# liudabao001/JABD-Joint-Attention-Based-Detector-for-small-face-detection

Measured on AMD Instinct MI355X. Metric: images/sec at 1024x1024 bs32 (1/2/4/8 GPU); boxes/sec NMS, higher is better.
Workload: dtype fp32; 1 GPU; C2: JABD-MobileNetV3 RetinaFace (nets/retinaface_r.py) eval forward, weights_init weights; global_batch=32, image_size=1024, parallelism=replicas x1

## Files before the change

jabd-joint-attention-based-detector-for-small-face-detection_amd/csrc/conv32.hip:

```cpp
#include <stdlib.h>

#include <algorithm>
#include <type_traits>

#include "common.h"
#include "conv_args.h"

namespace jabd {

typedef float f32x16 __attribute__((ext_vector_type(16)));

__device__ __forceinline__ float act32(float v, int act, float slope) {
  switch (act) {
    case ACT_RELU: return relu_f(v);
    case ACT_LEAKY: return v > 0.f ? v : v * slope;
    case ACT_HSWISH: return hswish_f(v);
    case ACT_HSIGMOID: return hsigmoid_f(v);
    case ACT_SIGMOID: return 1.f / (1.f + expf(-v));
    default: return v;
  }
}

constexpr int kBK = 32;

__device__ __forceinline__ void wave_lds_sync32() {
  asm volatile("s_waitcnt lgkmcnt(0)" ::: "memory");
  __builtin_amdgcn_wave_barrier();
}
constexpr int kG = kBK / 8;
constexpr int kGateLds = 1024;

constexpr int kEpiPitch = 36;
enum { kEpiRt = 0, kEpiNone = 1, kEpiRes = 2 };
template <int TN, bool ST, bool BB, int EPI = kEpiRt>
__device__ __forceinline__ void m32_epilogue_tm1(const ConvArgs& p, const f32x16 (&acc)[TN],
                                                 int pm, int om, int nb, int srow, float* ep,
                                                 float* __restrict__ part, const BnEpi& bb,
                                                 int lane, int ch0 = 0) {
  const bool has_bias = EPI == kEpiRt && p.bias;
  const bool has_res = EPI == kEpiRes || (EPI == kEpiRt && p.res);
  const int h = lane >> 5, j = lane & 31;
  const int ep_px = lane >> 3, ep_q = lane & 7;
  int mrow[4], prow[4];
#pragma unroll
  for (int r = 0; r < 4; ++r) {
    prow[r] = __shfl(pm, ep_px + 8 * r);
    mrow[r] = __shfl(om, ep_px + 8 * r);
  }
#pragma unroll
  for (int u = 0; u < TN; ++u) {
    const int nb0 = (nb * TN + u) * 32 + ch0;
    if (nb0 >= p.Cout) break;
    const int n = nb0 + 4 * ep_q;
    float4 ss = make_float4(0.f, 0.f, 0.f, 0.f), sq = ss, sh = ss;
    float4 bmu = sh, bis = sh, bgm = sh, bbt = sh;
    float4 bx[4], bmk[4];
    if constexpr (BB) {
      if (n < p.Cout) {
        bmu = *reinterpret_cast<const float4*>(bb.mean + n);
        bis = *reinterpret_cast<const float4*>(bb.invstd + n);
        if (!bb.mask) {
          bgm = *reinterpret_cast<const float4*>(bb.gamma + n);
          bbt = *reinterpret_cast<const float4*>(bb.beta + n);
        }
      }
#pragma unroll
      for (int r = 0; r < 4; ++r)
        bx[r] = (prow[r] >= 0 && n < p.Cout)
                    ? *reinterpret_cast<const float4*>(bb.x + (int64_t)mrow[r] * bb.x_ps + n)
                    : sh;
      if (bb.mask) {
#pragma unroll
        for (int r = 0; r < 4; ++r)
          bmk[r] = (prow[r] >= 0 && n < p.Cout)
                       ? *reinterpret_cast<const float4*>(bb.mask + (int64_t)mrow[r] * bb.mask_ps + n)
                       : sh;
      }
    }
#pragma unroll
    for (int c = 0; c < 4; ++c)
      *reinterpret_cast<float4*>(ep + j * kEpiPitch + 8 * c + 4 * h) =
          make_float4(acc[u][4 * c], acc[u][4 * c + 1], acc[u][4 * c + 2],
                      acc[u][4 * c + 3]);
    wave_lds_sync32();
    if constexpr (ST) sh = *reinterpret_cast<const float4*>(ep + 4 * ep_q);
#pragma unroll
    for (int r = 0; r < 4; ++r) {
      const int px = ep_px + 8 * r;
      if (prow[r] < 0 || n >= p.Cout) continue;
      float4 v = *reinterpret_cast<const float4*>(ep + px * kEpiPitch + 4 * ep_q);
      if (BB && bb.mask) {
        if (p.res) {
          const float4 rr = *reinterpret_cast<const float4*>(p.res + (int64_t)mrow[r] * p.res_ps +
                                                             p.res_c0 + n);
          v.x += rr.x; v.y += rr.y; v.z += rr.z; v.w += rr.w;
        }
        v.x *= bmk[r].x > 0.f ? 1.f : 0.f;
        v.y *= bmk[r].y > 0.f ? 1.f : 0.f;
        v.z *= bmk[r].z > 0.f ? 1.f : 0.f;
        v.w *= bmk[r].w > 0.f ? 1.f : 0.f;
        const float xh0 = (bx[r].x - bmu.x) * bis.x, xh1 = (bx[r].y - bmu.y) * bis.y;
        const float xh2 = (bx[r].z - bmu.z) * bis.z, xh3 = (bx[r].w - bmu.w) * bis.w;
        ss.x += v.x; ss.y += v.y; ss.z += v.z; ss.w += v.w;
        sq.x += v.x * xh0; sq.y += v.y * xh1; sq.z += v.z * xh2; sq.w += v.w * xh3;
        *reinterpret_cast<float4*>(p.y + (int64_t)mrow[r] * p.y_ps + p.y_c0 + n) = v;
        continue;
      }
      if constexpr (BB) {
        const float xv[4] = {bx[r].x, bx[r].y, bx[r].z, bx[r].w};
        const float mu[4] = {bmu.x, bmu.y, bmu.z, bmu.w}, is[4] = {bis.x, bis.y, bis.z, bis.w};
        const float gm[4] = {bgm.x, bgm.y, bgm.z, bgm.w}, bt[4] = {bbt.x, bbt.y, bbt.z, bbt.w};
        const float gv[4] = {v.x, v.y, v.z, v.w};
        float dzs[4], dzx[4];
#pragma unroll
        for (int e = 0; e < 4; ++e) {
          const float xh = (xv[e] - mu[e]) * is[e];
          const float z = fmaf(xh, gm[e], bt[e]);
          const float d = bb.act == ACT_RELU ? (z > 0.f ? 1.f : 0.f)
                          : bb.act == ACT_LEAKY ? (z > 0.f ? 1.f : bb.slope) : 1.f;
          dzs[e] = gv[e] * d;
          dzx[e] = dzs[e] * xh;
        }
        ss.x += dzs[0]; ss.y += dzs[1]; ss.z += dzs[2]; ss.w += dzs[3];
        sq.x += dzx[0]; sq.y += dzx[1]; sq.z += dzx[2]; sq.w += dzx[3];
      }
      if constexpr (ST) {
        const float dx = v.x - sh.x, dy = v.y - sh.y, dz = v.z - sh.z, dw = v.w - sh.w;
        ss.x += dx; ss.y += dy; ss.z += dz; ss.w += dw;
        sq.x = fmaf(dx, dx, sq.x); sq.y = fmaf(dy, dy, sq.y);
        sq.z = fmaf(dz, dz, sq.z); sq.w = fmaf(dw, dw, sq.w);
      }
      if (has_bias) {
        const float4 bb = *reinterpret_cast<const float4*>(p.bias + n);
        v.x += bb.x; v.y += bb.y; v.z += bb.z; v.w += bb.w;
      }
      if (has_res) {
        const float4 rr = *reinterpret_cast<const float4*>(p.res + (int64_t)mrow[r] * p.res_ps +
                                                           p.res_c0 + n);
        v.x += rr.x; v.y += rr.y; v.z += rr.z; v.w += rr.w;
      }
      if constexpr (EPI == kEpiRt) {
        v.x = act32(v.x, p.act, p.slope);
        v.y = act32(v.y, p.act, p.slope);
        v.z = act32(v.z, p.act, p.slope);
        v.w = act32(v.w, p.act, p.slope);
      }
      *reinterpret_cast<float4*>(p.y + (int64_t)mrow[r] * p.y_ps + p.y_c0 + n) = v;
    }
    if constexpr (BB) {
#pragma unroll
      for (int off = 8; off <= 32; off <<= 1) {
        ss.x += __shfl_xor(ss.x, off); ss.y += __shfl_xor(ss.y, off);
        ss.z += __shfl_xor(ss.z, off); ss.w += __shfl_xor(ss.w, off);
        sq.x += __shfl_xor(sq.x, off); sq.y += __shfl_xor(sq.y, off);
        sq.z += __shfl_xor(sq.z, off); sq.w += __shfl_xor(sq.w, off);
      }
      if (ep_px == 0 && (int64_t)srow * 32 < p.M && n < p.Cout) {
        const int ldc = p.Ntiles * 32;
        float* pr = bb.rows + (int64_t)srow * 2 * ldc + n;
        *reinterpret_cast<float4*>(pr) = ss;
        *reinterpret_cast<float4*>(pr + ldc) = sq;
      }
    }
    if constexpr (ST) {
#pragma unroll
      for (int off = 8; off <= 32; off <<= 1) {
        ss.x += __shfl_xor(ss.x, off); ss.y += __shfl_xor(ss.y, off);
        ss.z += __shfl_xor(ss.z, off); ss.w += __shfl_xor(ss.w, off);
        sq.x += __shfl_xor(sq.x, off); sq.y += __shfl_xor(sq.y, off);
        sq.z += __shfl_xor(sq.z, off); sq.w += __shfl_xor(sq.w, off);
      }
      const int64_t cnt = min<int64_t>(32, p.M - (int64_t)srow * 32);
      if (ep_px == 0 && cnt > 0 && n < p.Cout) {
        const float inv = 1.f / (float)cnt;
        const int ldc = p.Ntiles * 32;
        float* pr = part + (int64_t)srow * 2 * ldc + n;
        *reinterpret_cast<float4*>(pr) =
            make_float4(fmaf(ss.x, inv, sh.x), fmaf(ss.y, inv, sh.y), fmaf(ss.z, inv, sh.z),
                        fmaf(ss.w, inv, sh.w));
        *reinterpret_cast<float4*>(pr + ldc) =
            make_float4(fmaxf(sq.x - ss.x * ss.x * inv, 0.f), fmaxf(sq.y - ss.y * ss.y * inv, 0.f),
                        fmaxf(sq.z - ss.z * ss.z * inv, 0.f), fmaxf(sq.w - ss.w * ss.w * inv, 0.f));
      }
    }
    wave_lds_sync32();
  }
}

enum { kSrcRt = 0, kSrcOne = 1, kSrcTwo = 2 };
template <int TM, int TN, bool KXK, bool AS, bool ST = false, bool BB = false, int EPI = kEpiRt,
          int SRC = kSrcRt>
__global__ __launch_bounds__(256, 2) void conv1x1_m32_kernel(const ConvArgs p, int mtiles_img,
                                                             int per_img, int phase, int ks,
                                                             float* __restrict__ part,
                                                             const BnEpi bb) {
  constexpr bool FAST = SRC != kSrcRt;
  static_assert(!FAST || (AS && !KXK), "SRC: the gated 1x1 forms only");
  constexpr int BM = 4 * 32 * TM;
  constexpr int NB4 = kG * TN * 64;
  constexpr int NBT = (NB4 + 255) / 256;
  constexpr int kEpi4 = 4 * 32 * kEpiPitch / 4;
  constexpr int SB4 = (TM == 1 && kEpi4 > 2 * NB4) ? kEpi4 : 2 * NB4;
  __shared__ float4 sB_[SB4];
  float4 (*sB)[NB4] = reinterpret_cast<float4 (*)[NB4]>(sB_);
  __shared__ __attribute__((aligned(16))) float sGate[AS ? kGateLds : 4];
  const int lane = threadIdx.x & 63, wave = threadIdx.x >> 6;
  const int h = lane >> 5, j = lane & 31;
  const int nblk_n = p.Ntiles / TN;
  const int bid = blockIdx.x;
  const int nb = bid % nblk_n, mb = bid / nblk_n;
  const int OHW = p.OH * p.OW;
  const int ph = phase >> 1, pw = phase & 1;
  const int SH = phase >= 0 ? (p.OH - ph + 1) >> 1 : p.OH;
  const int SW = phase >= 0 ? (p.OW - pw + 1) >> 1 : p.OW;
  const int kh0 = phase >= 0 ? (ph + p.pad) & 1 : 0, kw0 = phase >= 0 ? (pw + p.pad) & 1 : 0;
  const int nkh = phase >= 0 ? (p.KH - kh0 + 1) >> 1 : p.KH;
  const int nkw = phase >= 0 ? (p.KW - kw0 + 1) >> 1 : p.KW;
  const int M = phase >= 0 ? p.B * SH * SW : (int)p.M;
  int img = 0, m_lo, m_hi;
  if (per_img) {
    img = mb / mtiles_img;
    m_lo = img * OHW + (mb - img * mtiles_img) * BM;
    m_hi = min(img * OHW + OHW, M);
  } else {
    m_lo = mb * BM;
    m_hi = M;
  }
  int pm[TM];
#pragma unroll
  for (int t = 0; t < TM; ++t) {
    const int m = m_lo + wave * 32 * TM + t * 32 + j;
    pm[t] = m < m_hi ? m : -1;
  }
  const int Kt = KXK ? nkh * nkw * p.Cin
                     : p.Cin + ((FAST ? SRC == kSrcTwo : p.x2 != nullptr) ? p.Cin2 : 0);
  const int S_all = (Kt + kBK - 1) / kBK;
  const int kchunk = (S_all + ks - 1) / ks;
  const int s_beg = ks > 1 ? (int)blockIdx.y * kchunk : 0;
  const int S = ks > 1 ? min(S_all, s_beg + kchunk) : S_all;
  int poh[TM], pow_[TM], om[TM];
  int64_t pbase[TM];
#pragma unroll
  for (int t = 0; t < TM; ++t) om[t] = pm[t];
  if constexpr (KXK) {
#pragma unroll
    for (int t = 0; t < TM; ++t) {
      const int m = pm[t] >= 0 ? pm[t] : 0;
      const int SHW = SH * SW;
      const int b = m / SHW, r = m - b * SHW;
      const int i = r / SW, jj = r - i * SW;
      poh[t] = phase >= 0 ? 2 * i + ph : i;
      pow_[t] = phase >= 0 ? 2 * jj + pw : jj;
      pbase[t] = (int64_t)b * p.x_bs + p.x_c0;
      if (pm[t] >= 0) om[t] = (b * p.OH + poh[t]) * p.OW + pow_[t];
    }
  }
  const int cps = p.Cin / kBK;
  const int x2_pix = (p.x2 && p.x2_stride != 1) ? (int)(p.x2_bs / p.x2_ps) : 0;
  const float4* wg = reinterpret_cast<const float4*>(p.w);
  const float* sc = AS ? p.ascale + (int64_t)img * p.ascale_bs : nullptr;

  const float* xa[TM];
  const float* xb[TM];
  if constexpr (FAST) {
#pragma unroll
    for (int t = 0; t < TM; ++t) {
      const int ml = pm[t] >= 0 ? pm[t] : m_lo;
      xa[t] = p.x + (int64_t)ml * p.x_ps + p.x_c0;
      xb[t] = SRC == kSrcTwo ? p.x2 + (int64_t)ml * p.x2_ps - p.Cin : xa[t];
    }
  }
  auto load_a = [&](int s, float4 (&a)[TM][kG]) {
    if constexpr (FAST) {
#pragma unroll
      for (int t = 0; t < TM; ++t)
#pragma unroll
        for (int q = 0; q < kG; ++q) {
          const int k4 = min(s * kBK + 8 * q + 4 * h, Kt - 4);
          const float* src = (SRC == kSrcTwo && k4 >= p.Cin) ? xb[t] + k4 : xa[t] + k4;
          a[t][q] = *reinterpret_cast<const float4*>(src);
        }
      return;
    }
    if constexpr (KXK) {
      const int tl = s / cps, ci0 = (s - tl * cps) * kBK;
      const int khi = tl / nkw;
      const int kh = kh0 + (phase >= 0 ? 2 : 1) * khi;
      const int kw = kw0 + (phase >= 0 ? 2 : 1) * (tl - khi * nkw);
#pragma unroll
      for (int t = 0; t < TM; ++t) {
        const int ih = p.tconv ? (poh[t] + p.pad - kh) >> (phase >= 0 ? 1 : 0)
                               : poh[t] * p.stride - p.pad + kh;
        const int iw = p.tconv ? (pow_[t] + p.pad - kw) >> (phase >= 0 ? 1 : 0)
                               : pow_[t] * p.stride - p.pad + kw;
        const bool ok = pm[t] >= 0 && ih >= 0 && ih < p.H && iw >= 0 && iw < p.W;
        const float* src = p.x + pbase[t] + ((int64_t)ih * p.W + iw) * p.x_ps + ci0 + 4 * h;
#pragma unroll
        for (int q = 0; q < kG; ++q)
          a[t][q] = ok ? *reinterpret_cast<const float4*>(src + 8 * q)
                       : make_float4(0.f, 0.f, 0.f, 0.f);
      }
      return;
    }
#pragma unroll
    for (int t = 0; t < TM; ++t)
#pragma unroll
      for (int q = 0; q < kG; ++q) {
        const int k4 = s * kBK + 8 * q + 4 * h;
        const int m = pm[t];
        float4 r = make_float4(0.f, 0.f, 0.f, 0.f);
        if (m >= 0) {
          if (k4 < p.Cin) {
            r = *reinterpret_cast<const float4*>(p.x + (int64_t)m * p.x_ps + p.x_c0 + k4);
          } else if (k4 < Kt) {
            int qq = m;
            if (p.x2_stride != 1) {
              const int b = m / OHW, rr = m - b * OHW;
              const int oh = rr / p.OW, ow = rr - oh * p.OW;
              qq = b * x2_pix + (oh * p.x2_stride) * p.x2_W + ow * p.x2_stride;
            }
            r = *reinterpret_cast<const float4*>(p.x2 + (int64_t)qq * p.x2_ps + (k4 - p.Cin));
          }
        }
        a[t][q] = r;
      }
  };
  const bool gate_lds = FAST || (AS && p.Cin <= kGateLds);
  auto zero_tail = [&](int s, float4 (&a)[TM][kG]) {
    if (!FAST || (s + 1) * kBK <= Kt) return;
#pragma unroll
    for (int t = 0; t < TM; ++t)
#pragma unroll
      for (int q = 0; q < kG; ++q)
        if (s * kBK + 8 * q + 4 * h >= Kt) a[t][q] = make_float4(0.f, 0.f, 0.f, 0.f);
  };
  auto load_b = [&](int s, float4 (&b)[NBT]) {
    if (KXK && phase >= 0) {
      const int tl = s / cps, khi = tl / nkw;
      const int tap = (kh0 + 2 * khi) * p.KW + kw0 + 2 * (tl - khi * nkw);
      s = tap * cps + (s - tl * cps);
    }
#pragma unroll
    for (int i = 0; i < NBT; ++i) {
      const int f = i * 256 + threadIdx.x;
      float4 v = make_float4(0.f, 0.f, 0.f, 0.f);
      if (f < NB4) {
        const int g = f / (TN * 64), rem = f - g * (TN * 64);
        const int u = rem >> 6, l = rem & 63;
        const int k8 = s * kG + g;
        v = wg[((int64_t)k8 * p.Ntiles + nb * TN + u) * 64 + l];
        if (!FAST && sc && !gate_lds) {
          int k0 = 8 * k8 + 4 * (l >> 5);
          if (KXK) k0 -= (s / cps) * p.Cin;
          if (k0 < p.Cin) {
            const float4 s4 = *reinterpret_cast<const float4*>(sc + k0);
            v.x *= s4.x; v.y *= s4.y; v.z *= s4.z; v.w *= s4.w;
          }
        }
      }
      b[i] = v;
    }
  };
  auto store_b = [&](int buf, int s, const float4 (&b)[NBT]) {
    if (KXK && phase >= 0) {
      const int tl = s / cps, khi = tl / nkw;
      const int tap = (kh0 + 2 * khi) * p.KW + kw0 + 2 * (tl - khi * nkw);
      s = tap * cps + (s - tl * cps);
    }
#pragma unroll
    for (int i = 0; i < NBT; ++i) {
      const int f = i * 256 + threadIdx.x;
      if (f < NB4) {
        float4 v = b[i];
        if (gate_lds) {
          const int g = f / (TN * 64), l = f & 63;
          int k0 = 8 * (s * kG + g) + 4 * (l >> 5);
          if (KXK) k0 -= (s / cps) * p.Cin;
          if (k0 < p.Cin) {
            const float4 s4 = *reinterpret_cast<const float4*>(sGate + k0);
            v.x *= s4.x; v.y *= s4.y; v.z *= s4.z; v.w *= s4.w;
          }
        }
        sB[buf][f] = v;
      }
    }
  };

  f32x16 acc[TM][TN];
#pragma unroll
  for (int t = 0; t < TM; ++t)
#pragma unroll
    for (int u = 0; u < TN; ++u)
#pragma unroll
      for (int r = 0; r < 16; ++r) acc[t][u][r] = 0.f;

  float4 a_cur[TM][kG], a_nxt[TM][kG], b_nxt[NBT];
  if (gate_lds) {
    for (int i = threadIdx.x; i < p.Cin; i += 256) sGate[i] = sc[i];
    __syncthreads();
  }
  if (S > s_beg) {
    load_a(s_beg, a_cur);
    load_b(s_beg, b_nxt);
    store_b(s_beg & 1, s_beg, b_nxt);
    zero_tail(s_beg, a_cur);
  }
  __syncthreads();
  for (int s = s_beg; s < S; ++s) {
    const bool more = s + 1 < S;
    if (more) {
      load_a(s + 1, a_nxt);
      load_b(s + 1, b_nxt);
    }
    const float4* bs = sB[s & 1];
#pragma unroll
    for (int q = 0; q < kG; ++q) {
      float4 bw[TN];
#pragma unroll
      for (int u = 0; u < TN; ++u) bw[u] = bs[(q * TN + u) * 64 + lane];
#pragma unroll
      for (int t = 0; t < TM; ++t)
#pragma unroll
        for (int u = 0; u < TN; ++u)
          acc[t][u] = __builtin_amdgcn_mfma_f32_32x32x2f32(bw[u].x, a_cur[t][q].x, acc[t][u], 0, 0, 0);
#pragma unroll
      for (int t = 0; t < TM; ++t)
#pragma unroll
        for (int u = 0; u < TN; ++u)
          acc[t][u] = __builtin_amdgcn_mfma_f32_32x32x2f32(bw[u].y, a_cur[t][q].y, acc[t][u], 0, 0, 0);
#pragma unroll
      for (int t = 0; t < TM; ++t)
#pragma unroll
        for (int u = 0; u < TN; ++u)
          acc[t][u] = __builtin_amdgcn_mfma_f32_32x32x2f32(bw[u].z, a_cur[t][q].z, acc[t][u], 0, 0, 0);
#pragma unroll
      for (int t = 0; t < TM; ++t)
#pragma unroll
        for (int u = 0; u < TN; ++u)
          acc[t][u] = __builtin_amdgcn_mfma_f32_32x32x2f32(bw[u].w, a_cur[t][q].w, acc[t][u], 0, 0, 0);
    }
    if (more) {
      store_b((s + 1) & 1, s + 1, b_nxt);
#pragma unroll
      for (int t = 0; t < TM; ++t)
#pragma unroll
        for (int q = 0; q < kG; ++q) a_cur[t][q] = a_nxt[t][q];
      zero_tail(s + 1, a_cur);
    }
    __syncthreads();
  }

  if (ks > 1) {
    const int npad = p.Ntiles * 32;
    float* pb = part + (int64_t)blockIdx.y * p.M * npad;
#pragma unroll
    for (int t = 0; t < TM; ++t) {
      if (pm[t] < 0) continue;
      float* prow = pb + (int64_t)om[t] * npad;
#pragma unroll
      for (int u = 0; u < TN; ++u)
#pragma unroll
        for (int c = 0; c < 4; ++c) {
          const int n = (nb * TN + u) * 32 + 8 * c + 4 * h;
          *reinterpret_cast<float4*>(prow + n) = make_float4(
              acc[t][u][4 * c], acc[t][u][4 * c + 1], acc[t][u][4 * c + 2], acc[t][u][4 * c + 3]);
        }
    }
    return;
  }
  if constexpr (TM == 1) {
    float* ep = reinterpret_cast<float*>(sB_) + wave * 32 * kEpiPitch;
    const int srow = mb * 4 + wave;
    m32_epilogue_tm1<TN, ST, BB, (ST || BB) ? kEpiNone : EPI>(p, acc[0], pm[0], om[0], nb, srow,
                                                                ep, part, bb, lane);
    return;
  }
#pragma unroll
  for (int t = 0; t < TM; ++t) {
    const int m = om[t];
    if (pm[t] < 0) continue;
    float* yrow = p.y + (int64_t)m * p.y_ps + p.y_c0;
    const float* rrow = p.res ? p.res + (int64_t)m * p.res_ps + p.res_c0 : nullptr;
#pragma unroll
    for (int u = 0; u < TN; ++u)
#pragma unroll
      for (int c = 0; c < 4; ++c) {
        const int n = (nb * TN + u) * 32 + 8 * c + 4 * h;
        if (n >= p.Cout) continue;
        float4 v = make_float4(acc[t][u][4 * c], acc[t][u][4 * c + 1], acc[t][u][4 * c + 2],
                               acc[t][u][4 * c + 3]);
        if (p.bias) {
          const float4 bb = *reinterpret_cast<const float4*>(p.bias + n);
          v.x += bb.x; v.y += bb.y; v.z += bb.z; v.w += bb.w;
        }
        if (rrow) {
          const float4 rr = *reinterpret_cast<const float4*>(rrow + n);
          v.x += rr.x; v.y += rr.y; v.z += rr.z; v.w += rr.w;
        }
        v.x = act32(v.x, p.act, p.slope);
        v.y = act32(v.y, p.act, p.slope);
        v.z = act32(v.z, p.act, p.slope);
        v.w = act32(v.w, p.act, p.slope);
        *reinterpret_cast<float4*>(yrow + n) = v;
      }
  }

}

__global__ __launch_bounds__(256) void m32_ksplit_reduce(const ConvArgs p, int ks,
                                                         const float* __restrict__ part) {
  const int npad = p.Ntiles * 32, c4n = (p.Cout + 3) >> 2;
  const int64_t i = blockIdx.x * (int64_t)blockDim.x + threadIdx.x;
  if (i >= p.M * c4n) return;
  const int64_t m = i / c4n;
  const int n = (int)(i - m * c4n) * 4;
  float4 v = *reinterpret_cast<const float4*>(part + m * npad + n);
  for (int y = 1; y < ks; ++y) {
    const float4 q = *reinterpret_cast<const float4*>(part + ((int64_t)y * p.M + m) * npad + n);
    v.x += q.x; v.y += q.y; v.z += q.z; v.w += q.w;
  }
  if (p.bias) {
    const float4 bb = *reinterpret_cast<const float4*>(p.bias + n);
    v.x += bb.x; v.y += bb.y; v.z += bb.z; v.w += bb.w;
  }
  if (p.res) {
    const float4 rr = *reinterpret_cast<const float4*>(p.res + m * p.res_ps + p.res_c0 + n);
    v.x += rr.x; v.y += rr.y; v.z += rr.z; v.w += rr.w;
  }
  v.x = act32(v.x, p.act, p.slope);
  v.y = act32(v.y, p.act, p.slope);
  v.z = act32(v.z, p.act, p.slope);
  v.w = act32(v.w, p.act, p.slope);
  *reinterpret_cast<float4*>(p.y + m * p.y_ps + p.y_c0 + n) = v;
}

template <int TN, bool AS, bool X2>
__global__ __launch_bounds__(512) void conv1x1_m32w8_kernel(const ConvArgs p, int mtiles_img,
                                                            int per_img) {
  constexpr int TNL = (TN + 1) / 2, TNH = TN - TNL;
  constexpr int NB4 = kG * TN * 64;
  constexpr int NBT = (NB4 + 511) / 512;
  constexpr int kEpi4 = 8 * 32 * kEpiPitch / 4;
  constexpr int SB4 = kEpi4 > 2 * NB4 ? kEpi4 : 2 * NB4;
  __shared__ float4 sB_[SB4];
  float4 (*sB)[NB4] = reinterpret_cast<float4 (*)[NB4]>(sB_);
  __shared__ __attribute__((aligned(16))) float sGate[AS ? kGateLds : 4];
  const int lane = threadIdx.x & 63;
  const int wave = __builtin_amdgcn_readfirstlane(threadIdx.x >> 6);
  const int row = wave & 3, half = wave >> 2;
  const int h = lane >> 5, j = lane & 31;
  const int nblk_n = p.Ntiles / TN;
  const int bid = blockIdx.x;
  const int nb = bid % nblk_n, mb = bid / nblk_n;
  const int OHW = p.OH * p.OW;
  int img = 0, m_lo, m_hi;
  if (per_img) {
    img = mb / mtiles_img;
    m_lo = img * OHW + (mb - img * mtiles_img) * 128;
    m_hi = min(img * OHW + OHW, (int)p.M);
  } else {
    m_lo = mb * 128;
    m_hi = (int)p.M;
  }
  const int m = m_lo + row * 32 + j;
  const int pm = m < m_hi ? m : -1;
  const int ml = pm >= 0 ? m : m_lo;
  const int Kt = p.Cin + (X2 ? p.Cin2 : 0);
  const int S = (Kt + kBK - 1) / kBK;
  const float4* wg = reinterpret_cast<const float4*>(p.w) + (int64_t)nb * TN * 64;
  const float* xa = p.x + (int64_t)ml * p.x_ps + p.x_c0;
  const float* xb = X2 ? p.x2 + (int64_t)ml * p.x2_ps - p.Cin : xa;

  auto load_a = [&](int s, float4 (&a)[kG]) {
#pragma unroll
    for (int q = 0; q < kG; ++q) {
      const int k4 = min(s * kBK + 8 * q + 4 * h, Kt - 4);
      const float* src = (X2 && k4 >= p.Cin) ? xb + k4 : xa + k4;
      a[q] = *reinterpret_cast<const float4*>(src);
    }
  };
  auto load_b = [&](int s, float4 (&b)[NBT]) {
#pragma unroll
    for (int i = 0; i < NBT; ++i) {
      const int f = i * 512 + threadIdx.x;
      if ((i + 1) * 512 <= NB4 || wave < (NB4 - i * 512) / 64) {
        const int g = f / (TN * 64), rem = f - g * (TN * 64);
        b[i] = wg[(int64_t)(s * kG + g) * p.Ntiles * 64 + rem];
      }
    }
  };
  auto store_b = [&](int buf, int s, const float4 (&b)[NBT]) {
#pragma unroll
    for (int i = 0; i < NBT; ++i) {
      const int f = i * 512 + threadIdx.x;
      if ((i + 1) * 512 <= NB4 || wave < (NB4 - i * 512) / 64) {
        float4 v = b[i];
        if constexpr (AS) {
          const int g = f / (TN * 64), l = f & 63;
          const int k0 = 8 * (s * kG + g) + 4 * (l >> 5);
          if (k0 < p.Cin) {
            const float4 s4 = *reinterpret_cast<const float4*>(sGate + k0);
            v.x *= s4.x; v.y *= s4.y; v.z *= s4.z; v.w *= s4.w;
          }
        }
        sB[buf][f] = v;
      }
    }
  };

  f32x16 acc[TNL];
#pragma unroll
  for (int u = 0; u < TNL; ++u)
#pragma unroll
    for (int r = 0; r < 16; ++r) acc[u][r] = 0.f;

  float4 a_cur[kG], a_nxt[kG], b_nxt[NBT];
  load_a(0, a_cur);
  load_b(0, b_nxt);
  if constexpr (AS) {
    const float* sc = p.ascale + (int64_t)img * p.ascale_bs;
    for (int i = threadIdx.x; i < p.Cin; i += 512) sGate[i] = sc[i];
    __syncthreads();
  }
  store_b(0, 0, b_nxt);
  auto zero_tail = [&](int s, float4 (&a)[kG]) {
    if ((s + 1) * kBK <= Kt) return;
#pragma unroll
    for (int q = 0; q < kG; ++q)
      if (s * kBK + 8 * q + 4 * h >= Kt) a[q] = make_float4(0.f, 0.f, 0.f, 0.f);
  };
  zero_tail(0, a_cur);
  __syncthreads();
  for (int s = 0; s < S; ++s) {
    const bool more = s + 1 < S;
    if (more) {
      load_a(s + 1, a_nxt);
      load_b(s + 1, b_nxt);
    }
    const float4* bs = sB[s & 1];
    auto mma = [&](auto nu_, auto u0_) {
      constexpr int NU = decltype(nu_)::value, U0 = decltype(u0_)::value;
#pragma unroll
      for (int q = 0; q < kG; ++q) {
        float4 bw[NU];
#pragma unroll
        for (int u = 0; u < NU; ++u) bw[u] = bs[(q * TN + U0 + u) * 64 + lane];
#pragma unroll
        for (int u = 0; u < NU; ++u)
          acc[u] = __builtin_amdgcn_mfma_f32_32x32x2f32(bw[u].x, a_cur[q].x, acc[u], 0, 0, 0);
#pragma unroll
        for (int u = 0; u < NU; ++u)
          acc[u] = __builtin_amdgcn_mfma_f32_32x32x2f32(bw[u].y, a_cur[q].y, acc[u], 0, 0, 0);
#pragma unroll
        for (int u = 0; u < NU; ++u)
          acc[u] = __builtin_amdgcn_mfma_f32_32x32x2f32(bw[u].z, a_cur[q].z, acc[u], 0, 0, 0);
#pragma unroll
        for (int u = 0; u < NU; ++u)
          acc[u] = __builtin_amdgcn_mfma_f32_32x32x2f32(bw[u].w, a_cur[q].w, acc[u], 0, 0, 0);
      }
    };
    if (half == 0)
      mma(std::integral_constant<int, TNL>{}, std::integral_constant<int, 0>{});
    else
      mma(std::integral_constant<int, TNH>{}, std::integral_constant<int, TNL>{});
    if (more) {
      store_b((s + 1) & 1, s + 1, b_nxt);
#pragma unroll
      for (int q = 0; q < kG; ++q) a_cur[q] = a_nxt[q];
      zero_tail(s + 1, a_cur);
    }
    __syncthreads();
  }

  float* ep = reinterpret_cast<float*>(sB_) + wave * 32 * kEpiPitch;
  if (half == 0)
    m32_epilogue_tm1<TNL, false, false, kEpiRt>(
        p, reinterpret_cast<const f32x16(&)[TNL]>(acc), pm, pm, 0, 0, ep, nullptr, BnEpi{}, lane,
        nb * TN * 32);
  else
    m32_epilogue_tm1<TNH, false, false, kEpiRt>(
        p, reinterpret_cast<const f32x16(&)[TNH]>(acc), pm, pm, 0, 0, ep, nullptr, BnEpi{}, lane,
        (nb * TN + TNL) * 32);
}

template <int TN, int KS, bool ST, bool BB, int EPI>
__global__ __launch_bounds__(256) void conv1x1_m32s_kernel(const ConvArgs p, int nblk_n,
                                                            float* __restrict__ part,
                                                            const BnEpi bb) {
  constexpr int NW4 = KS * kG * TN * 64;
  extern __shared__ __attribute__((aligned(16))) float4 m32s_lds[];
  const int lane = threadIdx.x & 63;
  const int wave = __builtin_amdgcn_readfirstlane(threadIdx.x >> 6);
  const int h = lane >> 5, j = lane & 31;
  const int xcd = blockIdx.x & 7, rr = blockIdx.x >> 3;
  const int nb = rr % nblk_n, wgm = (rr / nblk_n) * 8 + xcd;
  const int gm = gridDim.x / nblk_n;
  {
    const float4* wg = reinterpret_cast<const float4*>(p.w);
    for (int f = threadIdx.x; f < NW4; f += 256) {
      const int k8 = f / (TN * 64), rem = f - k8 * (TN * 64);
      m32s_lds[f] = wg[((int64_t)k8 * p.Ntiles + nb * TN + (rem >> 6)) * 64 + (rem & 63)];
    }
  }
  __syncthreads();
  float* ep = reinterpret_cast<float*>(m32s_lds + NW4) + wave * 32 * kEpiPitch;
  const int64_t ntiles = (p.M + 31) >> 5;
  const int64_t step = (int64_t)gm * 4;
  const float* xb = p.x + p.x_c0 + 4 * h;
  auto load = [&](int64_t T, int s, int q) {
    const int64_t m = T * 32 + j;
    return m < p.M ? *reinterpret_cast<const float4*>(xb + m * p.x_ps + s * kBK + 8 * q)
                   : make_float4(0.f, 0.f, 0.f, 0.f);
  };
  float4 a[KS][kG];
  int64_t T = (int64_t)wgm * 4 + wave;
#pragma unroll
  for (int s = 0; s < KS; ++s)
#pragma unroll
    for (int q = 0; q < kG; ++q) a[s][q] = load(T, s, q);
  for (; T < ntiles; T += step) {
    const int64_t Tn = T + step;
    f32x16 acc[TN];
#pragma unroll
    for (int u = 0; u < TN; ++u)
#pragma unroll
      for (int r = 0; r < 16; ++r) acc[u][r] = 0.f;
#pragma unroll
    for (int s = 0; s < KS; ++s)
#pragma unroll
      for (int q = 0; q < kG; ++q) {
        float4 bw[TN];
#pragma unroll
        for (int u = 0; u < TN; ++u) bw[u] = m32s_lds[((s * kG + q) * TN + u) * 64 + lane];
#pragma unroll
        for (int u = 0; u < TN; ++u)
          acc[u] = __builtin_amdgcn_mfma_f32_32x32x2f32(bw[u].x, a[s][q].x, acc[u], 0, 0, 0);
#pragma unroll
        for (int u = 0; u < TN; ++u)
          acc[u] = __builtin_amdgcn_mfma_f32_32x32x2f32(bw[u].y, a[s][q].y, acc[u], 0, 0, 0);
#pragma unroll
        for (int u = 0; u < TN; ++u)
          acc[u] = __builtin_amdgcn_mfma_f32_32x32x2f32(bw[u].z, a[s][q].z, acc[u], 0, 0, 0);
#pragma unroll
        for (int u = 0; u < TN; ++u)
          acc[u] = __builtin_amdgcn_mfma_f32_32x32x2f32(bw[u].w, a[s][q].w, acc[u], 0, 0, 0);
        a[s][q] = load(Tn, s, q);
      }
    const int64_t m = T * 32 + j;
    const int pm = m < p.M ? (int)m : -1;
    m32_epilogue_tm1<TN, ST, BB, EPI>(p, acc, pm, pm, nb, (int)T, ep, part, bb, lane);
  }
}

static int m32_ksplit(const ConvArgs& a, bool kxk, int64_t grid) {
  if (a.tconv || a.Cout % 4 || a.Cin % kBK || grid >= 256) return 1;
  const int Kt = kxk ? a.KH * a.KW * a.Cin : a.Cin + (a.x2 ? a.Cin2 : 0);
  const int S = (Kt + kBK - 1) / kBK;
  int ks = (int)std::min<int64_t>(8, (512 + grid - 1) / grid);
  ks = std::min(ks, S / 4);
  return ks >= 2 ? ks : 1;
}
static int64_t m32_ksplit_bytes(const ConvArgs& a, int ks) {
  return ks > 1 ? (int64_t)ks * a.B * a.OH * a.OW * a.ntiles32 * 32 * (int64_t)sizeof(float) : 0;
}
static int64_t m32_grid(const ConvArgs& a, int TM, int TN) {
  const int64_t BM = 4 * 32 * TM;
  const int64_t OHW = (int64_t)a.OH * a.OW;
  const int64_t mtiles = a.ascale ? cdiv(OHW, BM) * a.B : cdiv(a.M, BM);
  return mtiles * (a.ntiles32 / TN);
}

static bool m32_w8(const ConvArgs& a, int64_t grid) {
  static const bool off = env_digit("JABD_M32_W8") == 0;
  if (off || a.tconv || (a.ascale && a.Cin > kGateLds) || (a.x2 && a.x2_stride != 1))
    return false;
  static int ncu = 0;
  if (ncu <= 0) {
    int dev = 0;
    if (hipGetDevice(&dev) != hipSuccess ||
        hipDeviceGetAttribute(&ncu, hipDeviceAttributeMultiprocessorCount, dev) != hipSuccess)
      ncu = 0;
  }
  return grid < 2 * (int64_t)ncu;
}

template <int TM, int TN, bool KXK, bool AS>
static int launch_m32_as(const ConvArgs& a, int ks, hipStream_t st) {
  constexpr int BM = 4 * 32 * TM;
  const int64_t OHW = (int64_t)a.OH * a.OW;
  const int per_img = a.ascale != nullptr;
  const int64_t mt_img = cdiv(OHW, BM);
  if (KXK && a.tconv && a.stride == 2) {
    JABD_REQUIRE(!per_img, "conv32: phase mode without ascale");
    for (int ph = 0; ph < 2; ++ph)
      for (int pw = 0; pw < 2; ++pw) {
        const int64_t Mp = (int64_t)a.B * ((a.OH - ph + 1) / 2) * ((a.OW - pw + 1) / 2);
        if (Mp <= 0) continue;
        const int64_t grid = cdiv(Mp, BM) * (a.Ntiles / TN);
        JABD_REQUIRE(grid < (int64_t)0x7fffffff, "conv32: grid too large");
        conv1x1_m32_kernel<TM, TN, KXK, AS><<<(unsigned)grid, 256, 0, st>>>(a, (int)mt_img, 0,
                                                                        2 * ph + pw, 1, nullptr,
                                                                        BnEpi{});
        if (int e = check_launch("conv1x1_m32", 100 * TM + TN)) return e;
      }
    return JABD_OK;
  }
  const int64_t grid = m32_grid(a, TM, TN);
  JABD_REQUIRE(grid < (int64_t)0x7fffffff, "conv32: grid too large");
  if (ks > 1 && a.ws && a.ws_bytes >= m32_ksplit_bytes(a, ks)) {
    float* part = static_cast<float*>(a.ws);
    conv1x1_m32_kernel<TM, TN, KXK, AS><<<dim3((unsigned)grid, (unsigned)ks), 256, 0, st>>>(
        a, (int)mt_img, per_img, -1, ks, part, BnEpi{});
    if (int e = check_launch("conv1x1_m32 (split K)", 100 * TM + TN)) return e;
    const int64_t n4 = a.M * ((a.Cout + 3) / 4);
    m32_ksplit_reduce<<<(unsigned)cdiv(n4, 256), 256, 0, st>>>(a, ks, part);
    return check_launch("m32_ksplit_reduce");
  }
  if constexpr (TM == 1 && TN >= 5 && !KXK) {
    if (m32_w8(a, grid)) {
      if (a.x2)
        conv1x1_m32w8_kernel<TN, AS, true><<<(unsigned)grid, 512, 0, st>>>(a, (int)mt_img, per_img);
      else
        conv1x1_m32w8_kernel<TN, AS, false><<<(unsigned)grid, 512, 0, st>>>(a, (int)mt_img, per_img);
      return check_launch("conv1x1_m32", 100 * TM + TN);
    }
  }
  auto kern = conv1x1_m32_kernel<TM, TN, KXK, AS>;
  if constexpr (TM == 1 && !AS) {
    if (!a.bias && a.act == ACT_NONE)
      kern = a.res ? conv1x1_m32_kernel<1, TN, KXK, false, false, false, kEpiRes>
                   : conv1x1_m32_kernel<1, TN, KXK, false, false, false, kEpiNone>;
  }
  if constexpr (AS && !KXK) {
    if (a.Cin <= kGateLds && (!a.x2 || a.x2_stride == 1))
      kern = a.x2 ? conv1x1_m32_kernel<TM, TN, false, true, false, false, kEpiRt, kSrcTwo>
                  : conv1x1_m32_kernel<TM, TN, false, true, false, false, kEpiRt, kSrcOne>;
  }
  kern<<<(unsigned)grid, 256, 0, st>>>(a, (int)mt_img, per_img, -1, 1, nullptr, BnEpi{});
  return check_launch("conv1x1_m32", 100 * TM + TN);
}

template <int TM, int TN, bool KXK>
static int launch_m32(const ConvArgs& a, int ks, hipStream_t st) {
  if (a.ascale) return launch_m32_as<TM, TN, KXK, true>(a, ks, st);
  return launch_m32_as<TM, TN, KXK, false>(a, ks, st);
}

static bool m32s_on() {
  static const bool on = env_digit("JABD_M32S") != 0;
  return on;
}

template <int TN, int KS, bool ST, bool BB, int EPI>
static int launch_m32s(const ConvArgs& a, float* part, const BnEpi& bb, hipStream_t st) {
  auto kern = conv1x1_m32s_kernel<TN, KS, ST, BB, EPI>;
  const size_t lds = (size_t)KS * kG * TN * 64 * 16 + (size_t)4 * 32 * kEpiPitch * 4;
  static int slots = 0;
  if (slots <= 0) {
    int dev = 0, ncu = 0, occ = 0;
    JABD_HIP(hipGetDevice(&dev));
    JABD_HIP(hipDeviceGetAttribute(&ncu, hipDeviceAttributeMultiprocessorCount, dev));
    JABD_HIP(hipOccupancyMaxActiveBlocksPerMultiprocessor(&occ, kern, 256, lds));
    JABD_REQUIRE(occ >= 1, "conv32 stream: no resident workgroup (%zu B LDS)", lds);
    slots = ncu * occ;
  }
  const int nblk_n = a.Ntiles / TN;
  const int64_t ntiles = cdiv(a.M, (int64_t)32);
  int64_t gm = std::min<int64_t>(cdiv(ntiles, 4), slots / nblk_n);
  gm = std::max<int64_t>(8, gm / 8 * 8);
  kern<<<(unsigned)(gm * nblk_n), 256, lds, st>>>(a, nblk_n, part, bb);
  return check_launch("conv1x1_m32s", 100 * KS + TN);
}

bool m32s_pick(const ConvLayer& L, int form, int& TN, int& KS) {
  const ConvArgs& a = L.a;
  if (!m32s_on() || !L.is1x1 || a.tconv || a.nchw_in || a.x2 || a.ascale || a.y2 ||
      a.Cin % kBK || a.M >= ((int64_t)1 << 31) - 64)
    return false;
  KS = a.Cin / kBK;
  if (KS != 2 && KS != 4) return false;
  static const int ks4 = (int)env_int("JABD_M32S_KS4", 1);
  static const int ks2 = (int)env_int("JABD_M32S_KS2", 7);
  if (!(((KS == 4 ? ks4 : ks2) >> form) & 1)) return false;
  TN = a.tn32;
  while (KS * TN > 8 && TN % 2 == 0) TN /= 2;
  return TN >= 1 && KS * TN <= 8 && a.ntiles32 % TN == 0;
}

static int m32s_launch(const ConvArgs& a, int TN, int KS, int form, float* part, const BnEpi& bb,
                       hipStream_t st) {
  const bool plain_none = !a.bias && !a.res && a.act == ACT_NONE;
  const bool plain_res = !a.bias && a.res && a.act == ACT_NONE;
#define M32S(TN_, KS_)                                                                 \
  if (TN == TN_ && KS == KS_)                                                          \
  return form == 1   ? launch_m32s<TN_, KS_, true, false, kEpiNone>(a, part, bb, st)   \
         : form == 2 ? launch_m32s<TN_, KS_, false, true, kEpiNone>(a, part, bb, st)   \
         : plain_none ? launch_m32s<TN_, KS_, false, false, kEpiNone>(a, part, bb, st) \
         : plain_res  ? launch_m32s<TN_, KS_, false, false, kEpiRes>(a, part, bb, st)  \
                      : launch_m32s<TN_, KS_, false, false, kEpiRt>(a, part, bb, st);
  M32S(1, 2) M32S(2, 2) M32S(3, 2) M32S(4, 2) M32S(1, 4) M32S(2, 4)
#undef M32S
  return -1;
}

template <int TN, bool KXK>
static int launch_m32_stats(const ConvArgs& a, float* part, const BnEpi& bb, hipStream_t st) {
  const int64_t grid = cdiv(a.M, (int64_t)128) * (a.Ntiles / TN);
  JABD_REQUIRE(grid < (int64_t)0x7fffffff, "conv32 stats: grid too large");
  if (bb.rows) {
    conv1x1_m32_kernel<1, TN, KXK, false, false, true><<<(unsigned)grid, 256, 0, st>>>(
        a, (int)cdiv((int64_t)a.OH * a.OW, 128), 0, -1, 1, nullptr, bb);
    return check_launch("conv1x1_m32 (BN backward sums)", 100 + TN);
  }
  conv1x1_m32_kernel<1, TN, KXK, false, true><<<(unsigned)grid, 256, 0, st>>>(
      a, (int)cdiv((int64_t)a.OH * a.OW, 128), 0, -1, 1, part, BnEpi{});
  return check_launch("conv1x1_m32 (BN statistics)", 100 + TN);
}

int conv_m32_stats_dispatch(const ConvLayer& L, bool kxk, float* part, const BnEpi& bb,
                            hipStream_t st) {
  const ConvArgs a = L.view32();
  const int form = bb.rows ? 2 : 1;
  int tn, ks;
  if (!kxk && m32s_pick(L, form, tn, ks)) return m32s_launch(a, tn, ks, form, part, bb, st);
#define MS(TN_) return kxk ? launch_m32_stats<TN_, true>(a, part, bb, st) : launch_m32_stats<TN_, false>(a, part, bb, st);
  switch (a.tn32) {
    case 1: MS(1)
    case 2: MS(2)
    case 3: MS(3)
    case 4: MS(4)
    default: return -1;
  }
#undef MS
}

}

using namespace jabd;

static int m32_tm(const ConvArgs& a) {
  static const int ftm = (int)env_int("JABD_M32_TM", 0);
  if (a.tn32 > 4) return 1;
  if (ftm == 1 || ftm == 2) return ftm;
  return (!a.ascale || a.M < 65536) ? 1 : 2;
}

static int m32_tn_launch(const ConvArgs& a) {
  static const bool off = env_digit("JABD_M32_TN1") == 0;
  if (off || a.tn32 <= 1 || a.tconv || !a.ascale) return a.tn32;
  return m32_grid(a, m32_tm(a), a.tn32) >= 256 ? a.tn32 : 1;
}

namespace jabd {
bool m32_tile_pick(const ConvLayer& L, int& tm, int& tn, int& ks) {
  const ConvArgs& a = L.a;
  if (!L.w32(1, 7)) return false;
  if (L.is1x1 ? !L.fast1x1
              : !(L.v4out && !a.x2 && !a.y2 && L.kxk32() &&
                  (!a.tconv || a.stride == 1 || (a.stride == 2 && !a.ascale))))
    return false;
  tn = m32_tn_launch(a);
  tm = (tn == 1 && a.tn32 > 1) ? 1 : m32_tm(a);
  ks = m32_ksplit(a, !L.is1x1, m32_grid(a, tm, tn));
  return true;
}

int64_t conv_m32_ksplit_bytes(const ConvArgs& a, int ks) { return m32_ksplit_bytes(a, ks); }

int conv_m32s_launch(const ConvLayer& L, const ConvRoute& r, hipStream_t st) {
  return m32s_launch(L.view32(), r.tn, r.ks, 0, nullptr, BnEpi{}, st);
}

int conv_m32_tile_launch(const ConvLayer& L, const ConvRoute& r, hipStream_t st) {
  const ConvArgs a = L.view32();
  const bool kxk = !L.is1x1;
#define M32(TM_, TN_)             \
  if (r.tm == TM_ && r.tn == TN_) \
    return kxk ? launch_m32<TM_, TN_, true>(a, r.ks, st) : launch_m32<TM_, TN_, false>(a, r.ks, st);
  M32(1, 1) M32(1, 2) M32(1, 3) M32(1, 4) M32(2, 1) M32(2, 2) M32(2, 3) M32(2, 4)
  M32(1, 5) M32(1, 6) M32(1, 7)
#undef M32
  return -1;
}
}

extern "C" int jabd_conv_pack_tn32(int cout) {
  const int nt = (cout + 31) / 32;
  if (nt <= 4) return nt;
  if (nt % 4 == 0) return 4;
  int best = 4, waste = (nt + 3) / 4 * 4 - nt;
  for (int tn : {5, 6, 7}) {
    const int w = (nt + tn - 1) / tn * tn - nt;
    if (w < waste) { waste = w; best = tn; }
  }
  return best;
}

namespace jabd {

__device__ __forceinline__ float w2d_at(const float* __restrict__ w, int cout, int cin, int khw,
                                        int transposed, int k, int n) {
  const int cinp = transposed ? cout : cin;
  const int ncols = transposed ? cin : cout;
  if (k >= khw * cinp || n >= ncols) return 0.f;
  const int tap = k / cinp, c = k - tap * cinp;
  const int co = transposed ? c : n, ci = transposed ? n : c;
  return w[((int64_t)co * cin + ci) * khw + tap];
}

__device__ __forceinline__ void pack_store16(const float* __restrict__ w, int cout, int cin,
                                             int khw, int tr, int Ntiles, float* __restrict__ wp,
                                             int64_t i) {
  const int lane = (int)(i & 63);
  const int64_t r = i >> 6;
  const int nt = (int)(r % Ntiles), kc = (int)(r / Ntiles);
  const int g = lane >> 4, j = lane & 15;
  float4 v;
  v.x = w2d_at(w, cout, cin, khw, tr, 16 * kc + 4 * g + 0, 16 * nt + j);
  v.y = w2d_at(w, cout, cin, khw, tr, 16 * kc + 4 * g + 1, 16 * nt + j);
  v.z = w2d_at(w, cout, cin, khw, tr, 16 * kc + 4 * g + 2, 16 * nt + j);
  v.w = w2d_at(w, cout, cin, khw, tr, 16 * kc + 4 * g + 3, 16 * nt + j);
  reinterpret_cast<float4*>(wp)[i] = v;
}

__device__ __forceinline__ void pack_store32(const float* __restrict__ w, int cout, int cin,
                                             int khw, int tr, int NT32, float* __restrict__ wp32,
                                             int64_t i) {
  const int lane = (int)(i & 63);
  const int64_t r = i >> 6;
  const int nt = (int)(r % NT32), k8 = (int)(r / NT32);
  const int h = lane >> 5, j = lane & 31;
  float4 v;
  v.x = w2d_at(w, cout, cin, khw, tr, 8 * k8 + 4 * h + 0, 32 * nt + j);
  v.y = w2d_at(w, cout, cin, khw, tr, 8 * k8 + 4 * h + 1, 32 * nt + j);
  v.z = w2d_at(w, cout, cin, khw, tr, 8 * k8 + 4 * h + 2, 32 * nt + j);
  v.w = w2d_at(w, cout, cin, khw, tr, 8 * k8 + 4 * h + 3, 32 * nt + j);
  reinterpret_cast<float4*>(wp32)[i] = v;
}

__global__ __launch_bounds__(256) void pack_w_kernel(const float* __restrict__ w, int cout,
                                                     int cin, int khw, int transposed, int Kc,
                                                     int Ntiles, float* __restrict__ wp, int K8,
                                                     int NT32, float* __restrict__ wp32) {
  const int64_t i = blockIdx.x * (int64_t)blockDim.x + threadIdx.x;
  const int64_t n16 = (int64_t)Kc * Ntiles * 64;
  if (i < n16)
    pack_store16(w, cout, cin, khw, transposed, Ntiles, wp, i);
  else if (wp32 && i - n16 < (int64_t)K8 * NT32 * 64)
    pack_store32(w, cout, cin, khw, transposed, NT32, wp32, i - n16);
}

constexpr int kPackMaxJobs = 1024;
__global__ __launch_bounds__(256) void pack_w_multi_kernel(const int64_t* __restrict__ jobs,
                                                           const int64_t* __restrict__ starts,
                                                           int njobs, int64_t total) {
  __shared__ int64_t st[kPackMaxJobs + 1];
  for (int t = threadIdx.x; t <= njobs; t += blockDim.x) st[t] = starts[t];
  __syncthreads();
  const int64_t i = blockIdx.x * (int64_t)blockDim.x + threadIdx.x;
  if (i >= total) return;
  int lo = 0, hi = njobs - 1;
  while (lo < hi) {
    const int mid = (lo + hi + 1) >> 1;
    if (st[mid] <= i) lo = mid; else hi = mid - 1;
  }
  const int64_t* jb = jobs + (int64_t)lo * 11;
  const float* w = reinterpret_cast<const float*>(jb[0]);
  float* wp = reinterpret_cast<float*>(jb[1]);
  float* wp32 = reinterpret_cast<float*>(jb[2]);
  const int cout = (int)jb[3], cin = (int)jb[4], khw = (int)jb[5], tr = (int)jb[6];
  const int Kc = (int)jb[7], Ntiles = (int)jb[8], NT32 = (int)jb[10];
  const int64_t r0 = i - st[lo];
  const int64_t n16 = (int64_t)Kc * Ntiles * 64;
  if (r0 < n16)
    pack_store16(w, cout, cin, khw, tr, Ntiles, wp, r0);
  else
    pack_store32(w, cout, cin, khw, tr, NT32, wp32, r0 - n16);
}

}

extern "C" int jabd_conv_pack_multi_f32(const int64_t* jobs, const int64_t* starts,
                                        int32_t njobs, int64_t total, jabd_stream_t stream) {
  using namespace jabd;
  if (njobs <= 0 || total <= 0) return JABD_OK;
  JABD_REQUIRE(jobs && starts && njobs <= kPackMaxJobs, "conv_pack_multi: bad args (njobs %d)",
               njobs);
  pack_w_multi_kernel<<<(unsigned)cdiv(total, 256), 256, 0, as_stream(stream)>>>(jobs, starts,
                                                                                njobs, total);
  return check_launch("conv_pack_multi");
}

extern "C" int jabd_conv_pack_f32(const float* w, int32_t cout, int32_t cin, int32_t kh,
                                  int32_t kw, int32_t transposed, int32_t Kc, int32_t Ntiles,
                                  float* wp, int32_t K8, int32_t NT32, float* wp32,
                                  jabd_stream_t stream) {
  using namespace jabd;
  JABD_REQUIRE(w && wp && cout > 0 && cin > 0 && kh > 0 && kw > 0 && Kc > 0 && Ntiles > 0 &&
                   (!wp32 || (K8 > 0 && NT32 > 0)),
               "conv_pack: bad args");
  const int cinp = transposed ? cout : cin, ncols = transposed ? cin : cout;
  JABD_REQUIRE(16 * Kc >= kh * kw * cinp && 16 * Ntiles >= ncols &&
                   (!wp32 || (8 * K8 >= kh * kw * cinp && 32 * NT32 >= ncols)),
               "conv_pack: tile counts do not cover the weight");
  const int64_t tot = (int64_t)Kc * Ntiles * 64 + (wp32 ? (int64_t)K8 * NT32 * 64 : 0);
  pack_w_kernel<<<(unsigned)cdiv(tot, 256), 256, 0, as_stream(stream)>>>(
      w, cout, cin, kh * kw, transposed, Kc, Ntiles, wp, K8, NT32, wp32);
  return check_launch("conv_pack");
}
```

Before: 5204 images/sec.

## Add software-pipelined gated 1x1 MFMA tile with interior/tail stage split

Introduces a shared device routine for the gated (attention-scaled) 1x1 conv forms. It double-buffers A fragments and B weight tiles across K steps and applies the gate scale when staging weights into LDS. It also splits the K loop into interior stages without bounds checks and a general tail, with sched_barriers around the MFMA block. Both the 4-wave kernel (for selected TM/TN) and the 8-wave kernel route their gated variants through it, aiming to overlap global loads with MFMA and cut per-step branch overhead. The cost is higher register pressure from the duplicated A buffers and a new code path for these shapes.

```diff
diff --git a/jabd-joint-attention-based-detector-for-small-face-detection_amd/csrc/conv32.hip b/jabd-joint-attention-based-detector-for-small-face-detection_amd/csrc/conv32.hip
--- a/jabd-joint-attention-based-detector-for-small-face-detection_amd/csrc/conv32.hip
+++ b/jabd-joint-attention-based-detector-for-small-face-detection_amd/csrc/conv32.hip
@@ -188,6 +188,254 @@
 }
 
 enum { kSrcRt = 0, kSrcOne = 1, kSrcTwo = 2 };
+
+constexpr bool m32_gated_stepped(int tm, int tn) {
+  return tn == 3 || tn == 4 || (tm == 1 && tn == 2);
+}
+
+template <int TM, int TN, int SRC, bool W8>
+__device__ __forceinline__ void m32_gated_tile(const ConvArgs& p, int mtiles_img, int per_img) {
+  static_assert(!W8 || TM == 1, "the 8-wave form has 32-pixel wave tiles");
+  constexpr int NWV = W8 ? 8 : 4;
+  constexpr int BM = 4 * 32 * TM;
+  constexpr int TNL = W8 ? (TN + 1) / 2 : TN;
+  constexpr int TNH = TN - TNL;
+  constexpr int NB4 = kG * TN * 64;
+  constexpr int NBT = (kG * TN + NWV - 1) / NWV;
+  constexpr int kEpi4 = NWV * 32 * kEpiPitch / 4;
+  constexpr int SB4 = (TM == 1 && kEpi4 > 2 * NB4) ? kEpi4 : 2 * NB4;
+  __shared__ float4 sB_[SB4];
+  float4 (*sB)[NB4] = reinterpret_cast<float4 (*)[NB4]>(sB_);
+  __shared__ __attribute__((aligned(16))) float sGate[kGateLds];
+  const int lane = threadIdx.x & 63;
+  const int wave = __builtin_amdgcn_readfirstlane(threadIdx.x >> 6);
+  const int row = W8 ? wave & 3 : wave, half = W8 ? wave >> 2 : 0;
+  const int h = lane >> 5, j = lane & 31;
+  const int nblk_n = p.Ntiles / TN;
+  const int bid = blockIdx.x;
+  const int nb = bid % nblk_n, mb = bid / nblk_n;
+  const int OHW = p.OH * p.OW;
+  int img = 0, m_lo, m_hi;
+  if (per_img) {
+    img = mb / mtiles_img;
+    m_lo = img * OHW + (mb - img * mtiles_img) * BM;
+    m_hi = min(img * OHW + OHW, (int)p.M);
+  } else {
+    m_lo = mb * BM;
+    m_hi = (int)p.M;
+  }
+  int pm[TM];
+  const float* xa[TM];
+#pragma unroll
+  for (int t = 0; t < TM; ++t) {
+    const int m = m_lo + row * 32 * TM + t * 32 + j;
+    pm[t] = m < m_hi ? m : -1;
+    const int ml = pm[t] >= 0 ? m : m_lo;
+    xa[t] = p.x + (int64_t)ml * p.x_ps + p.x_c0 + 4 * h;
+  }
+  const int Kt = p.Cin + (SRC == kSrcTwo ? p.Cin2 : 0);
+  const int S = (Kt + kBK - 1) / kBK;
+  const int s_in = p.Cin / kBK;
+
+  int wgrp[NBT];
+  int64_t woff[NBT];
+#pragma unroll
+  for (int i = 0; i < NBT; ++i) {
+    const int w = i * NWV + wave;
+    wgrp[i] = w / TN;
+    woff[i] = ((int64_t)wgrp[i] * p.Ntiles + nb * TN + (w - wgrp[i] * TN)) * 64;
+  }
+  const float4* wg = reinterpret_cast<const float4*>(p.w);
+  const int64_t wstep = (int64_t)kG * p.Ntiles * 64;
+  auto live_b = [&](int i) {
+    return (i + 1) * NWV <= kG * TN || wave < kG * TN - i * NWV;
+  };
+  auto load_b = [&](int s, float4 (&b)[NBT]) {
+    const float4* ws = wg + s * wstep;
+#pragma unroll
+    for (int i = 0; i < NBT; ++i)
+      if (live_b(i)) b[i] = (ws + woff[i])[lane];
+  };
+  auto store_b = [&](auto interior, int buf, int s, const float4 (&b)[NBT]) {
+#pragma unroll
+    for (int i = 0; i < NBT; ++i)
+      if (live_b(i)) {
+        float4 v = b[i];
+        const int k0 = s * kBK + 8 * wgrp[i] + 4 * h;
+        if (decltype(interior)::value || k0 < p.Cin) {
+          const float4 s4 = *reinterpret_cast<const float4*>(sGate + k0);
+          v.x *= s4.x; v.y *= s4.y; v.z *= s4.z; v.w *= s4.w;
+        }
+        sB[buf][i * (NWV * 64) + threadIdx.x] = v;
+      }
+  };
+  auto load_a = [&](auto interior, int s, float4 (&a)[TM][kG]) {
+#pragma unroll
+    for (int t = 0; t < TM; ++t)
+#pragma unroll
+      for (int q = 0; q < kG; ++q) {
+        if constexpr (decltype(interior)::value) {
+          a[t][q] = *reinterpret_cast<const float4*>(xa[t] + s * kBK + 8 * q);
+        } else {
+          const int k4 = min(s * kBK + 8 * q + 4 * h, Kt - 4);
+          const float* src = xa[t];
+          if constexpr (SRC == kSrcTwo) {
+            const int ml = pm[t] >= 0 ? pm[t] : m_lo;
+            const float* xb = p.x2 + (int64_t)ml * p.x2_ps - p.Cin + 4 * h;
+            src = k4 >= p.Cin ? xb : src;
+          }
+          a[t][q] = *reinterpret_cast<const float4*>(src + (k4 - 4 * h));
+        }
+      }
+  };
+  auto zero_tail = [&](int s, float4 (&a)[TM][kG]) {
+    if ((s + 1) * kBK <= Kt) return;
+#pragma unroll
+    for (int t = 0; t < TM; ++t)
+#pragma unroll
+      for (int q = 0; q < kG; ++q)
+        if (s * kBK + 8 * q + 4 * h >= Kt) a[t][q] = make_float4(0.f, 0.f, 0.f, 0.f);
+  };
+
+  f32x16 acc[TM][TNL];
+#pragma unroll
+  for (int t = 0; t < TM; ++t)
+#pragma unroll
+    for (int u = 0; u < TNL; ++u)
+#pragma unroll
+      for (int r = 0; r < 16; ++r) acc[t][u][r] = 0.f;
+
+  auto mma_part = [&](const float4* bs, const float4 (&ac)[TM][kG], auto nu_, auto u0_) {
+    constexpr int NU = decltype(nu_)::value, U0 = decltype(u0_)::value;
+#pragma unroll
+    for (int q = 0; q < kG; ++q) {
+      float4 bw[NU];
+#pragma unroll
+      for (int u = 0; u < NU; ++u) bw[u] = bs[(q * TN + U0 + u) * 64 + lane];
+#pragma unroll
+      for (int t = 0; t < TM; ++t)
+#pragma unroll
+        for (int u = 0; u < NU; ++u)
+          acc[t][u] = __builtin_amdgcn_mfma_f32_32x32x2f32(bw[u].x, ac[t][q].x, acc[t][u], 0, 0, 0);
+#pragma unroll
+      for (int t = 0; t < TM; ++t)
+#pragma unroll
+        for (int u = 0; u < NU; ++u)
+          acc[t][u] = __builtin_amdgcn_mfma_f32_32x32x2f32(bw[u].y, ac[t][q].y, acc[t][u], 0, 0, 0);
+#pragma unroll
+      for (int t = 0; t < TM; ++t)
+#pragma unroll
+        for (int u = 0; u < NU; ++u)
+          acc[t][u] = __builtin_amdgcn_mfma_f32_32x32x2f32(bw[u].z, ac[t][q].z, acc[t][u], 0, 0, 0);
+#pragma unroll
+      for (int t = 0; t < TM; ++t)
+#pragma unroll
+        for (int u = 0; u < NU; ++u)
+          acc[t][u] = __builtin_amdgcn_mfma_f32_32x32x2f32(bw[u].w, ac[t][q].w, acc[t][u], 0, 0, 0);
+    }
+  };
+  auto mma = [&](const float4* bs, const float4 (&ac)[TM][kG]) {
+    if constexpr (W8) {
+      if (half == 0)
+        mma_part(bs, ac, std::integral_constant<int, TNL>{}, std::integral_constant<int, 0>{});
+      else
+        mma_part(bs, ac, std::integral_constant<int, TNH>{}, std::integral_constant<int, TNL>{});
+    } else {
+      mma_part(bs, ac, std::integral_constant<int, TN>{}, std::integral_constant<int, 0>{});
+    }
+  };
+
+  const std::true_type interior{};
+  const std::false_type general{};
+  float4 a[2][TM][kG], b_nxt[NBT];
+  const float* sc = p.ascale + (int64_t)img * p.ascale_bs;
+  if constexpr (W8) {
+    load_a(general, 0, a[0]);
+    load_b(0, b_nxt);
+  }
+  for (int i = threadIdx.x; i < p.Cin; i += NWV * 64) sGate[i] = sc[i];
+  __syncthreads();
+  if constexpr (!W8) {
+    load_a(general, 0, a[0]);
+    load_b(0, b_nxt);
+  }
+  store_b(general, 0, 0, b_nxt);
+  zero_tail(0, a[0]);
+  __syncthreads();
+  auto stage = [&](auto par, auto in, int s) {
+    constexpr int P = decltype(par)::value;
+    const bool more = decltype(in)::value || s + 1 < S;
+    if (more) {
+      load_a(in, s + 1, a[P ^ 1]);
+      load_b(s + 1, b_nxt);
+    }
+    __builtin_amdgcn_sched_barrier(0);
+    mma(sB[P], a[P]);
+    __builtin_amdgcn_sched_barrier(0);
+    if (more) {
+      store_b(in, P ^ 1, s + 1, b_nxt);
+      if constexpr (!decltype(in)::value) zero_tail(s + 1, a[P ^ 1]);
+    }
+    __syncthreads();
+  };
+  const std::integral_constant<int, 0> even{};
+  const std::integral_constant<int, 1> odd{};
+  int s = 0;
+  for (; s + 2 < s_in; s += 2) {
+    stage(even, interior, s);
+    stage(odd, interior, s + 1);
+  }
+  for (; s < S; s += 2) {
+    stage(even, general, s);
+    if (s + 1 < S) stage(odd, general, s + 1);
+  }
+
+  if constexpr (TM == 1) {
+    float* ep = reinterpret_cast<float*>(sB_) + wave * 32 * kEpiPitch;
+    if constexpr (!W8) {
+      m32_epilogue_tm1<TN, false, false, kEpiRt>(p, acc[0], pm[0], pm[0], nb, mb * 4 + wave, ep,
+                                                 nullptr, BnEpi{}, lane);
+    } else if (half == 0) {
+      m32_epilogue_tm1<TNL, false, false, kEpiRt>(p, acc[0], pm[0], pm[0], 0, 0, ep, nullptr,
+                                                  BnEpi{}, lane, nb * TN * 32);
+    } else {
+      m32_epilogue_tm1<TNH, false, false, kEpiRt>(
+          p, reinterpret_cast<const f32x16(&)[TNH]>(acc[0]), pm[0], pm[0], 0, 0, ep, nullptr,
+          BnEpi{}, lane, (nb * TN + TNL) * 32);
+    }
+    return;
+  }
+#pragma unroll
+  for (int t = 0; t < TM; ++t) {
+    const int m = pm[t];
+    if (m < 0) continue;
+    float* yrow = p.y + (int64_t)m * p.y_ps + p.y_c0;
+    const float* rrow = p.res ? p.res + (int64_t)m * p.res_ps + p.res_c0 : nullptr;
+#pragma unroll
+    for (int u = 0; u < TN; ++u)
+#pragma unroll
+      for (int c = 0; c < 4; ++c) {
+        const int n = (nb * TN + u) * 32 + 8 * c + 4 * h;
+        if (n >= p.Cout) continue;
+        float4 v = make_float4(acc[t][u][4 * c], acc[t][u][4 * c + 1], acc[t][u][4 * c + 2],
+                               acc[t][u][4 * c + 3]);
+        if (p.bias) {
+          const float4 bb = *reinterpret_cast<const float4*>(p.bias + n);
+          v.x += bb.x; v.y += bb.y; v.z += bb.z; v.w += bb.w;
+        }
+        if (rrow) {
+          const float4 rr = *reinterpret_cast<const float4*>(rrow + n);
+          v.x += rr.x; v.y += rr.y; v.z += rr.z; v.w += rr.w;
+        }
+        v.x = act32(v.x, p.act, p.slope);
+        v.y = act32(v.y, p.act, p.slope);
+        v.z = act32(v.z, p.act, p.slope);
+        v.w = act32(v.w, p.act, p.slope);
+        *reinterpret_cast<float4*>(yrow + n) = v;
+      }
+  }
+}
+
 template <int TM, int TN, bool KXK, bool AS, bool ST = false, bool BB = false, int EPI = kEpiRt,
           int SRC = kSrcRt>
 __global__ __launch_bounds__(256, 2) void conv1x1_m32_kernel(const ConvArgs p, int mtiles_img,
@@ -196,6 +444,11 @@
                                                              const BnEpi bb) {
   constexpr bool FAST = SRC != kSrcRt;
   static_assert(!FAST || (AS && !KXK), "SRC: the gated 1x1 forms only");
+  if constexpr (FAST && m32_gated_stepped(TM, TN)) {
+    static_assert(!ST && !BB && EPI == kEpiRt, "SRC: the plain epilogue only");
+    m32_gated_tile<TM, TN, SRC, false>(p, mtiles_img, per_img);
+    return;
+  }
   constexpr int BM = 4 * 32 * TM;
   constexpr int NB4 = kG * TN * 64;
   constexpr int NBT = (NB4 + 255) / 256;
@@ -537,6 +790,13 @@
 template <int TN, bool AS, bool X2>
 __global__ __launch_bounds__(512) void conv1x1_m32w8_kernel(const ConvArgs p, int mtiles_img,
                                                             int per_img) {
+  if constexpr (AS) {
+    if constexpr (X2)
+      m32_gated_tile<1, TN, kSrcTwo, true>(p, mtiles_img, per_img);
+    else
+      m32_gated_tile<1, TN, kSrcOne, true>(p, mtiles_img, per_img);
+    return;
+  }
   constexpr int TNL = (TN + 1) / 2, TNH = TN - TNL;
   constexpr int NB4 = kG * TN * 64;
   constexpr int NBT = (NB4 + 511) / 512;
```

Result: no change. 5243 images/sec (median of 6 runs) (+0.8%).
